# TopHillRobotics/quadruped-robot

Hardware: AMD Instinct MI355X
Metric: MPC+WBC control ticks/s (batched robots) (higher is better)
Workload: dtype f32 assembly / f64 QP+WBC

## Files before the change

quadruped-robot_amd/csrc/qrgpu_api.hip:

```cpp
#include <hip/hip_runtime.h>
#include <hip/hip_ext.h>
#include <cmath>
#include <cstdio>
#include <cstdlib>
#include <cstring>
#include <mutex>
#include <string>

#include "qrgpu_ctx.h"
#include "qr_wbc_model.h"

hipError_t create_side_stream(hipStream_t *s)
{
    int least = 0, greatest = 0;
    if (hipDeviceGetStreamPriorityRange(&least, &greatest) == hipSuccess && greatest != least)
        return hipStreamCreateWithPriority(s, hipStreamNonBlocking, greatest);
    return hipStreamCreateWithFlags(s, hipStreamNonBlocking);
}

static void lane_destroy(Lane &L);

int lane_create(qrgpu_ctx *c, Lane &L, bool own_stream, bool masked)
{
    if (L.d_order) return QRGPU_OK;
    L.own_stream = own_stream; L.masked = own_stream && masked;
    const size_t nb = (size_t)c->max_batch;
    auto zalloc = [](auto **p, size_t bytes) { return hipMalloc((void **)p, bytes) == hipSuccess && hipMemset(*p, 0, bytes) == hipSuccess; };
    bool ok = hipMalloc(&L.d_order, sizeof(int) * 2 * nb) == hipSuccess && zalloc(&L.d_rescue, sizeof(int) * (nb + 2)) && zalloc(&L.d_pre, sizeof(int) * (2 * nb + 4)) &&
              zalloc(&L.d_skip, nb) && hipHostMalloc((void **)&L.h_pre_count, 4 * sizeof(int), hipHostMallocMapped) == hipSuccess &&
              hipHostGetDevicePointer((void **)&L.d_pre_hint, L.h_pre_count, 0) == hipSuccess && zalloc(&L.d_started, sizeof(int)) &&
              ((own_stream && !masked) || masked || create_side_stream(&L.side_stream) == hipSuccess) && zalloc(&L.d_done_flag, sizeof(unsigned) * nb) && zalloc(&L.d_qhead, 16 * sizeof(int)) &&
              zalloc(&L.d_planned_done, sizeof(int)) && zalloc(&L.d_go, (1 + QR_ABORT_RING) * sizeof(int)) && zalloc(&L.d_lane_done, sizeof(int)) && zalloc(&L.d_main_done, sizeof(int)) && zalloc(&L.d_rescue_taken, 4 * sizeof(int)) &&
              hipMalloc(&L.d_cmd_tick, sizeof(float) * 12 * nb) == hipSuccess &&
              hipEventCreateWithFlags(&L.ev_fork, hipEventDisableTiming) == hipSuccess && hipEventCreateWithFlags(&L.ev_join, hipEventDisableTiming) == hipSuccess;
    if (ok && own_stream) {
        const uint32_t words = (uint32_t)((c->num_cu + 31) / 32);
        ok = (masked ? (hipExtStreamCreateWithCUMask(&L.stream, words, c->mask16_main) == hipSuccess && hipExtStreamCreateWithCUMask(&L.side_stream, words, c->mask16_side) == hipSuccess)
                     : hipStreamCreateWithFlags(&L.stream, hipStreamNonBlocking) == hipSuccess);
    }
    if (ok && masked) ok = hipMemset(L.d_rescue + 2, 0xff, sizeof(int) * nb) == hipSuccess;
    if (ok) { L.h_pre_count[0] = L.h_pre_count[1] = L.h_pre_count[2] = L.h_pre_count[3] = 0; }
    (void)hipDeviceSynchronize();
    if (!ok) lane_destroy(L);
    return ok ? QRGPU_OK : QRGPU_ERR_ALLOC;
}
static void lane_destroy(Lane &L)
{
    if (L.stream && L.own_stream) { (void)hipStreamSynchronize(L.stream); }
    if (L.side_stream && (!L.own_stream || L.masked)) { (void)hipStreamSynchronize(L.side_stream); hipStreamDestroy(L.side_stream); }
    if (L.stream && L.own_stream) hipStreamDestroy(L.stream);
    (void)hipHostFree(L.h_pre_count);
    for (void *p : {(void *)L.d_order, (void *)L.d_rescue, (void *)L.d_pre, (void *)L.d_skip, (void *)L.d_started, (void *)L.d_done_flag, (void *)L.d_qhead,
                    (void *)L.d_planned_done, (void *)L.d_go, (void *)L.d_lane_done, (void *)L.d_main_done, (void *)L.d_rescue_taken, (void *)L.d_cmd_tick})
        (void)hipFree(p);
    if (L.ev_fork) hipEventDestroy(L.ev_fork);
    if (L.ev_join) hipEventDestroy(L.ev_join);
    L = Lane{};
}

int upload_wbc(qrgpu_ctx *c)
{
    if (!c->wbc_dirty) return QRGPU_OK;
    HIPCHK(c, hipMemcpyAsync(c->d_wbc, c->wbc_host, sizeof(WbcConst) * QRGPU_MAX_TYPES, hipMemcpyHostToDevice, c->stream));
    HIPCHK(c, hipStreamSynchronize(c->stream));
    c->wbc_dirty = false;
    return QRGPU_OK;
}

int launch_wbc(qrgpu_ctx *c, int n, const int *d_type, const float *d_state, const float *d_cmd, float *d_prev, float *d_tau, float *d_qdes, int *d_status,
               const WbcOpts &o)
{
    if (!batch_ok(c, n) || !d_state) return QRGPU_ERR_BAD_ARG;
    if (!o.dbg && (!d_cmd || !d_prev || !d_tau)) return QRGPU_ERR_BAD_ARG;
    if (!(d_type ? ready_mask(c->wbc_ready) != 0 : c->wbc_ready[0])) return QRGPU_ERR_NOT_SETUP;
    HIPCHK(c, hipSetDevice(c->device));
    int rc = upload_wbc(c);
    if (rc) return rc;
    const hipStream_t ws = o.stream ? o.stream : c->stream;
    if (!o.pipe.wbc_done) c->ov_chain = false;
    {
        TimerScope ts(c, 1, ws, !o.pipe.second && o.timed);
        hipLaunchKernelGGL((o.dbg || o.qp || c->d_dbg_cycles_wbc) ? qr_wbc_kernel_dbg : qr_wbc_kernel, dim3(o.grid_wgs > 0 ? o.grid_wgs : 8 * ((n + 7) / 8)), dim3(128), 0, ws, n, c->d_wbc, d_type, d_state,
                           d_cmd ? d_cmd : d_state, d_prev, d_tau, d_qdes, d_status, o.dbg, o.merge, o.status_or, (long long *)c->d_dbg_cycles_wbc, o.fr,
                           ready_mask(c->wbc_ready), o.epilogue, o.qp, o.pipe);
    }
    HIPCHK(c, hipGetLastError());
    return QRGPU_OK;
}

int launch_vmc(qrgpu_ctx *c, int n, const int *d_type_id, const float *d_vmc_in, const float *d_ratio, const float *d_q, float *d_force,
               float *d_tau, int *d_status)
{
    if (!batch_ok(c, n) || !d_vmc_in || !d_force) return QRGPU_ERR_BAD_ARG;
    if (d_tau && !d_q) return QRGPU_ERR_BAD_ARG;
    if (!(d_type_id ? ready_mask(c->vmc_ready) != 0 : c->vmc_ready[0])) return QRGPU_ERR_NOT_SETUP;
    HIPCHK(c, hipSetDevice(c->device));
    VmcLaunch P = c->vmc;
    P.n = n; P.ratio = d_ratio; P.type_ready = ready_mask(c->vmc_ready);
    hipLaunchKernelGGL(qr_vmc_kernel, dim3(8 * ((n + 7) / 8)), dim3(64), 0, c->stream, P, d_type_id, d_vmc_in, d_q, d_force, d_tau, d_status);
    HIPCHK(c, hipGetLastError());
    return QRGPU_OK;
}

extern "C" {

void qrgpu_model_desc_default(qrgpu_model_desc *d)
{
    d->hip_l = 0.08505f; d->upper_l = 0.2f; d->lower_l = 0.2f;
    d->body_size[0] = 0.267f; d->body_size[1] = 0.194f; d->body_size[2] = 0.114f;
    d->kp_body_pos = 100.f; d->kd_body_pos = 10.f; d->kp_body_ori = 100.f; d->kd_body_ori = 10.f;
    d->kp_foot = 500.f; d->kd_foot = 10.f; d->weight_fb = 0.1f; d->weight_fr = 1.f; d->mu = 0.4f;
}

extern char **environ;
static void warn_unknown_env()
{
    static std::once_flag once;
    std::call_once(once, [] {
        static const char *supported[] = {QRGPU_SUPPORTED_ENV};
        static const char *labs[] = {QRGPU_LAB_ENV};
        const bool lab_on = lab_env("QRGPU_LAB") != nullptr;
        for (char **e = environ; e && *e; ++e) {
            if (strncmp(*e, "QRGPU_", 6) != 0 || strncmp(*e, "QRGPU_BENCH_", 12) == 0) continue;
            const char *eq = strchr(*e, '=');
            const std::string name(*e, eq ? (size_t)(eq - *e) : strlen(*e));
            bool ok = false, is_lab = false;
            for (const char *s_ : supported) if (name == s_) ok = true;
            for (const char *s_ : labs) if (name == s_) is_lab = true;
            if (ok || (is_lab && lab_on)) continue;
            if (is_lab) fprintf(stderr, "libqrgpu: %s is a laboratory switch: ignored unless QRGPU_LAB=1 is set (include/qrgpu.h lists the supported ones)\n", name.c_str());
            else fprintf(stderr, "libqrgpu: %s is not an environment switch of this library (include/qrgpu.h lists the supported ones): ignored\n", name.c_str());
        }
    });
}

int qrgpu_create(int device_id, int max_batch, int horizon_max, qrgpu_ctx **out)
{
    if (!out || max_batch <= 0 || horizon_max <= 0 || horizon_max > QRGPU_MAX_HORIZON) return QRGPU_ERR_BAD_ARG;
    warn_unknown_env();
    *out = nullptr;
    int ndev = 0;
    if (hipGetDeviceCount(&ndev) != hipSuccess || device_id < 0 || device_id >= ndev) return QRGPU_ERR_NO_DEVICE;
    if (hipSetDevice(device_id) != hipSuccess) return QRGPU_ERR_NO_DEVICE;
    hipDeviceProp_t prop;
    if (hipGetDeviceProperties(&prop, device_id) != hipSuccess) return QRGPU_ERR_NO_DEVICE;
    if (strncmp(prop.gcnArchName, "gfx950", 6) != 0) return QRGPU_ERR_NO_DEVICE;
    qrgpu_ctx *c = new qrgpu_ctx();
    c->device = device_id; c->max_batch = max_batch; c->horizon_max = horizon_max;
    c->name = prop.name; c->num_cu = prop.multiProcessorCount;
    c->lds_per_cu = (int)prop.maxSharedMemoryPerMultiProcessor;
    if (c->lds_per_cu <= 0) c->lds_per_cu = 160 * 1024;
    const size_t in1 = 28 + 12 * QRGPU_MAX_HORIZON + 4 * QRGPU_MAX_HORIZON + 12 + 37 + 67 + 3;
    static_assert(28 + 12 * QRGPU_MAX_HORIZON + 4 * QRGPU_MAX_HORIZON + 12 + 37 + 67 + 3 <= 512, "staging layout");
    c->zero_copy = !qr_env().single_copies;
    bool stage_ok;
    if (c->zero_copy) {
        void *dp = nullptr;
        stage_ok = hipHostMalloc(&c->h_stage, 640 * sizeof(float), hipHostMallocMapped) == hipSuccess &&
                   hipHostGetDevicePointer(&dp, c->h_stage, 0) == hipSuccess;
        if (stage_ok) {
            memset(c->h_stage, 0, 640 * sizeof(float));
            c->h_in1 = (float *)c->h_stage; c->h_out1 = c->h_in1 + 512; c->h_st1 = (int *)(c->h_in1 + 576);
            c->d_in1 = (float *)dp; c->d_out1 = c->d_in1 + 512; c->d_st1 = (int *)(c->d_in1 + 576);
        }
    } else {
        stage_ok = hipMalloc(&c->d_in1, in1 * sizeof(float)) == hipSuccess && hipMalloc(&c->d_out1, 64 * sizeof(float)) == hipSuccess &&
                   hipMalloc(&c->d_st1, 4 * sizeof(int)) == hipSuccess;
    }
    auto zalloc = [](auto **p, size_t bytes) { return hipMalloc((void **)p, bytes) == hipSuccess && hipMemset(*p, 0, bytes) == hipSuccess; };
    bool ok = stage_ok && hipMalloc(&c->d_wbc, sizeof(WbcConst) * QRGPU_MAX_TYPES) == hipSuccess;
    const size_t nb = (size_t)max_batch;
    ok = ok && zalloc(&c->d_body, sizeof(qrgpu_plant_body_desc) * QRGPU_MAX_TYPES);
    ok = ok && zalloc(&c->d_cost[0], sizeof(int) * nb) && zalloc(&c->d_cost[1], sizeof(int) * nb) && hipMalloc(&c->d_warm, (size_t)QR_WARM_STRIDE * nb) == hipSuccess &&
         hipStreamCreateWithFlags(&c->wbc_stream, hipStreamNonBlocking) == hipSuccess &&
         zalloc(&c->d_main_started, sizeof(int)) && zalloc(&c->d_tick_done, sizeof(int)) && zalloc(&c->d_gate_abort, QR_ABORT_RING * sizeof(int)) &&
         zalloc(&c->d_wbc_finished, sizeof(int)) && zalloc(&c->d_solved, sizeof(unsigned) * nb) && zalloc(&c->d_wbc_done, sizeof(unsigned) * nb) &&
         hipMalloc(&c->d_ftime, sizeof(int) * nb) == hipSuccess;
    ok = ok && lane_create(c, c->lane[0], false) == QRGPU_OK;
    if (!ok) {
        qrgpu_destroy(c);
        return QRGPU_ERR_ALLOC;
    }
    if (hipStreamCreateWithFlags(&c->own_stream, hipStreamNonBlocking) == hipSuccess) c->stream = c->own_stream;
    c->lane[0].stream = c->stream;
    (void)hipDeviceSynchronize();
    memset(&c->mpc, 0, sizeof(c->mpc));
    memset(c->wbc_host, 0, sizeof(c->wbc_host));
    *out = c;
    return QRGPU_OK;
}

void qrgpu_destroy(qrgpu_ctx *c)
{
    if (!c) return;
    hipSetDevice(c->device);
    (void)hipStreamSynchronize(c->stream);
    if (c->wbc_stream) (void)hipStreamSynchronize(c->wbc_stream);
    qrgpu_comm_destroy(c);
    for (int l = 0; l < QR_LANES; ++l) lane_destroy(c->lane[l]);
    for (int k = 0; k < 2; ++k) for (auto &e : c->ev[k]) { hipEventDestroy(e.first); hipEventDestroy(e.second); }
    for (auto &e : c->marks) hipEventDestroy(e);
    if (c->wbc_stream) hipStreamDestroy(c->wbc_stream);
    if (c->wbc_stream_hi) { (void)hipStreamSynchronize(c->wbc_stream_hi); hipStreamDestroy(c->wbc_stream_hi); }
    if (c->own_stream) hipStreamDestroy(c->own_stream);
    for (int k = 0; k < 2; ++k) if (c->ev_call[k]) hipEventDestroy(c->ev_call[k]);
    if (c->h_stage) (void)hipHostFree(c->h_stage);
    else for (void *p : {(void *)c->d_in1, (void *)c->d_out1, (void *)c->d_st1}) (void)hipFree(p);
    for (void *p : {(void *)c->d_wbc, (void *)c->d_body, (void *)c->d_cost[0], (void *)c->d_cost[1], (void *)c->d_warm, (void *)c->d_flops, (void *)c->d_main_started, (void *)c->d_ftime,
                    (void *)c->d_wbc_finished, (void *)c->d_gate_abort, (void *)c->d_solved, (void *)c->d_wbc_done, (void *)c->d_gather_done, (void *)c->d_tick_done,
                    (void *)c->d_timeline, (void *)c->d_tlr, (void *)c->d_sinv_spill, c->d_dbg_cycles, c->d_dbg_cycles_wbc, (void *)c->d_join_dbg})
        (void)hipFree(p);
    delete c;
}

static void forget_history(qrgpu_ctx *c)
{
    for (auto &L : c->lane) { L.lpt_n = 0; L.plan_n = 0; }
    c->cost_n[0] = c->cost_n[1] = 0;
    c->ov_hold = 0;
}
int qrgpu_set_lpt_schedule(qrgpu_ctx *c, int on)
{
    if (!c) return QRGPU_ERR_BAD_ARG;
    c->lpt = on != 0;
    forget_history(c);
    return QRGPU_OK;
}
int qrgpu_set_warm_start(qrgpu_ctx *c, int on)
{
    if (!c) return QRGPU_ERR_BAD_ARG;
    c->warm = on != 0;
    c->warm_n = 0;
    return QRGPU_OK;
}
int qrgpu_mpc_set_hessian_mode(qrgpu_ctx *c, int mode)
{
    if (!c || (mode != QRGPU_HESSIAN_F32 && mode != QRGPU_HESSIAN_BF16X3)) return QRGPU_ERR_BAD_ARG;
    c->mpc.hess_mode = mode;
    return QRGPU_OK;
}
int qrgpu_set_planned_list(qrgpu_ctx *c, int on, int big_nls)
{
    if (!c || big_nls < 0) return QRGPU_ERR_BAD_ARG;
    c->planned = on != 0;
    c->big_nls = big_nls;
    for (auto &L : c->lane) L.plan_n = 0;
    return QRGPU_OK;
}
int qrgpu_set_tick_pipeline(qrgpu_ctx *c, int on)
{
    if (!c) return QRGPU_ERR_BAD_ARG;
    c->pipeline = on != 0;
    return QRGPU_OK;
}
int qrgpu_set_rescue_pass(qrgpu_ctx *c, int on)
{
    if (!c) return QRGPU_ERR_BAD_ARG;
    c->rescue = on != 0;
    for (auto &L : c->lane) L.plan_n = 0;
    return QRGPU_OK;
}
int qrgpu_set_stream(qrgpu_ctx *c, void *s) { if (!c) return QRGPU_ERR_BAD_ARG; c->stream = (hipStream_t)s; c->lane[0].stream = c->stream; c->ov_chain = false; return QRGPU_OK; }
void *qrgpu_get_stream(qrgpu_ctx *c) { return c ? (void *)c->stream : nullptr; }
const char *qrgpu_last_error(const qrgpu_ctx *c) { return c ? c->err.c_str() : "null context"; }
int qrgpu_device_info(const qrgpu_ctx *c, char *name, int len, int *lds)
{
    if (!c) return 0;
    if (name && len > 0) { strncpy(name, c->name.c_str(), len - 1); name[len - 1] = 0; }
    if (lds) *lds = c->lds_per_cu;
    return c->num_cu;
}

int qrgpu_mpc_setup(qrgpu_ctx *c, int type_id, float dt, int horizon, float mu, float fmax, float mass,
                    const float inertia[3], const float weights[12], float alpha)
{
    if (!c || type_id < 0 || type_id >= QRGPU_MAX_TYPES || !inertia || !weights) return QRGPU_ERR_BAD_ARG;
    if (horizon <= 0 || horizon > c->horizon_max) return QRGPU_ERR_BAD_ARG;
    if (c->mpc.horizon != horizon) for (int t = 0; t < QRGPU_MAX_TYPES; ++t) if (t != type_id) c->mpc_ready[t] = false;
    MpcType &T = c->mpc.type[type_id];
    T.dt = dt; T.mu = mu; T.fmax = fmax; T.mass = mass; T.alpha = alpha;
    for (int i = 0; i < 3; ++i) T.inertia[i] = inertia[i];
    for (int i = 0; i < 12; ++i) T.weights[i] = weights[i];
    if (!c->wbc_ready[type_id]) { T.hip_l = 0.08505f; T.upper_l = 0.2f; T.lower_l = 0.2f; }
    c->mpc.horizon = horizon;
    c->mpc_ready[type_id] = true;
    return QRGPU_OK;
}

int qrgpu_wbc_setup(qrgpu_ctx *c, int type_id, const qrgpu_model_desc *desc)
{
    if (!c || type_id < 0 || type_id >= QRGPU_MAX_TYPES || !desc) return QRGPU_ERR_BAD_ARG;
    build_wbc_const(*desc, c->wbc_host[type_id]);
    MpcType &T = c->mpc.type[type_id];
    T.hip_l = desc->hip_l; T.upper_l = desc->upper_l; T.lower_l = desc->lower_l;
    c->wbc_ready[type_id] = true;
    c->wbc_dirty = true;
    return QRGPU_OK;
}

int qrgpu_mpc_solve_batch(qrgpu_ctx *c, int n, const int *d_type_id, const float *d_mpc_state, const float *d_traj,
                          const float *d_gait, const float *d_q, float *d_force, float *d_tau_mpc, int *d_status)
{
// ... 331 lines not shown
```

quadruped-robot_amd/csrc/qrgpu_ctx.h:

```cpp
#pragma once
#include <hip/hip_runtime.h>
#include <cstdlib>
#include <cstring>
#include <string>
#include <utility>
#include <vector>

#include "../../include/qrgpu.h"
#include "qr_device_types.h"
#include "qr_kernels.h"

using namespace qrgpu;

enum MpcVar {
    MPC_MAIN11,
    MPC_LIST11,
    MPC_ONE11,
    MPC_HALF_LIST11,
    MPC_MAIN16,
    MPC_LIST16,
    MPC_TWO16,
    MPC_PERSIST11,
    MPC_PERSIST16,
    MPC_VAR_COUNT,
    MPC_VAR_NONE = -1
};

#define QR_LANES 5
#define QR_ABORT_RING 8
struct Lane {
    hipStream_t stream = nullptr;
    bool own_stream = false;
    hipStream_t side_stream = nullptr;
    hipEvent_t ev_fork = nullptr, ev_join = nullptr;
    int *d_order = nullptr;
    int lpt_n = 0;
    int *d_rescue = nullptr;
    int rescue_parity = 0;
    bool last_rescue_active = false;
    int last_rescue_parity = 0;
    int *d_pre = nullptr;
    unsigned char *d_skip = nullptr;
    int plan_n = 0;
    int *d_pre_hint = nullptr;
    int *h_pre_count = nullptr;
    int plan_sync_left = 0;
    int *d_started = nullptr;
    unsigned started_total = 0;
    int *d_go = nullptr;
    unsigned go_total = 0;
    int plan_epoch = 0;
    int *d_planned_done = nullptr;
    unsigned planned_done_total = 0;
    int *d_qhead = nullptr;
    int qhead_parity = 0;
    int two_hold = 0;
    bool two_probe = false;
    unsigned *d_done_flag = nullptr;
    float *d_cmd_tick = nullptr;
    bool masked = false;
    int *d_lane_done = nullptr;
    int *d_main_done = nullptr; int main_done_total = 0;
    int order_parity = 0;
    const int *order_used = nullptr;
    bool join_recorded = false;
    int last_linger = 0;
    int *d_rescue_taken = nullptr;
    unsigned lane_done_total = 0;
};

struct qrgpu_ctx {
    int device = 0;
    int max_batch = 0;
    int horizon_max = 0;
    hipStream_t stream = nullptr;
    hipStream_t own_stream = nullptr;
    MpcLaunch mpc{};
    bool mpc_ready[QRGPU_MAX_TYPES] = {false, false, false, false};
    bool wbc_ready[QRGPU_MAX_TYPES] = {false, false, false, false};
    VmcLaunch vmc{};
    bool vmc_ready[QRGPU_MAX_TYPES] = {false, false, false, false};
    WbcConst wbc_host[QRGPU_MAX_TYPES];
    WbcConst *d_wbc = nullptr;
    bool wbc_dirty = true;
    qrgpu_plant_body_desc body_host[QRGPU_MAX_TYPES] = {};
    qrgpu_plant_body_desc *d_body = nullptr;
    bool body_ready[QRGPU_MAX_TYPES] = {false, false, false, false};
    bool body_dirty = true;
    qrgpu_stage_reset stage_reset{};
    bool stage_reset_on = false;
    float *d_in1 = nullptr;
    float *d_out1 = nullptr;
    int *d_st1 = nullptr;
    float *h_in1 = nullptr, *h_out1 = nullptr;
    int *h_st1 = nullptr;
    void *h_stage = nullptr;
    bool zero_copy = false;
    int type_stage = 0;
    Lane lane[QR_LANES];
    int *d_cost[2] = {nullptr, nullptr};
    int cost_n[2] = {0, 0};
    double *d_sinv_spill = nullptr;
    bool planned = true;
    int big_nls = 0;
    bool pipeline = true;
    hipStream_t wbc_stream = nullptr;
    int *d_main_started = nullptr;
    unsigned main_started_total = 0;
    unsigned tick_epoch = 0;
    int main_slots[MPC_VAR_COUNT] = {};
    int main_slots_lds[MPC_VAR_COUNT] = {};
    int *d_tick_done = nullptr;
    unsigned tick_done_total = 0;
    bool last_tick_piped = false;
    int *d_gather_done = nullptr;
    unsigned gather_total[2] = {0, 0};
    unsigned gather_joined[2] = {0, 0};
    int *d_gate_abort = nullptr;
    int *d_wbc_finished = nullptr;
    unsigned wbc_finished_total = 0;
    int overlap = 0;
    int ov_next = 0;
    bool ov_chain = false;
    int ov_n = 0;
    unsigned ov_epoch = 0, ov_main_total = 0;
    const void *ov_out[4] = {nullptr, nullptr, nullptr, nullptr};
    const void *ov_prev_ori = nullptr;
    int ov_lane_last = 0;
    int ov_fence_slots = 0;
    int ov_hold = 0;
    bool ov_prev_plan = false;
    hipStream_t wbc_stream_hi = nullptr;
    int ov16_side_cus = 0;
    uint32_t mask16_main[16] = {}, mask16_side[16] = {};
    hipEvent_t ev_call[2] = {nullptr, nullptr};
    int ev_call_last = -1;
    long long *d_join_dbg = nullptr;
    int ov_stats[2] = {0, 0};
    unsigned *d_solved = nullptr;
    unsigned *d_wbc_done = nullptr;
    int *d_tlr = nullptr;
    long long *d_timeline = nullptr;
    int *d_ftime = nullptr;
    bool lpt = true;
    bool rescue = true;
    int epilogue = 0;
    double *d_flops = nullptr;
    bool flops_on = false;
    int flops_n = 0;
    bool warm = true;
    unsigned char *d_warm = nullptr;
    int warm_n = 0;
    bool last_main_persist = false;
    void *d_dbg_cycles_wbc = nullptr;
    void *d_dbg_cycles = nullptr;
    int lds_per_cu = 0, num_cu = 0;
    std::string name;
    std::string err;
    void *comm = nullptr;
    bool comm_owned = false;
    int comm_nranks = 0, comm_rank = 0;
    hipStream_t comm_stream = nullptr;
    hipEvent_t ev_tick = nullptr;
    hipEvent_t ev_gather[2] = {nullptr, nullptr};
    bool ev_gather_pending[2] = {false, false};
    bool timing = false;
    bool timing_paused = false;
    int timing_every = 1;
    unsigned ev_calls[2] = {0, 0};
    std::vector<std::pair<hipEvent_t, hipEvent_t>> ev[2];
    size_t ev_used[2] = {0, 0};
    std::vector<hipEvent_t> marks;
};

inline const char *lab_env(const char *name)
{
    static const bool lab = [] { const char *e = getenv("QRGPU_LAB"); return e && atoi(e) != 0; }();
    return lab ? getenv(name) : nullptr;
}
#define QRGPU_SUPPORTED_ENV "QRGPU_TICK_PIPELINE", "QRGPU_PIPE_GATE_MS", "QRGPU_PLAN_GO_MS", "QRGPU_PIPE_WAIT_US", "QRGPU_OV_WAIT_US", "QRGPU_OV_FAULT", "QRGPU_OV_PLAN_HOLD", "QRGPU_OV16", \
                            "QRGPU_COMM_EVENTS", "QRGPU_SINGLE_COPIES", "QRGPU_PERSIST", "QRGPU_H16_TWO", "QRGPU_H16_TWO_HOLD", "QRGPU_H16_BIG_US", "QRGPU_H16_BIG_STAY_US", \
                            "QRGPU_LIB", "QRGPU_EXTRA_FLAGS", "QRGPU_LAB"
#define QRGPU_LAB_ENV "QRGPU_WBC_CHUNKS", "QRGPU_PLANNED_FORK"

struct QrEnv {
    static int num(const char *e, int dflt) { return e ? atoi(e) : dflt; }
    static long long ms(const char *e) { return 100000LL * (e ? atoll(e) : 50LL); }
    static long long us(const char *e, long long dflt_ticks) { return e ? 100LL * atoll(e) : dflt_ticks; }
    int tick_pipeline = num(getenv("QRGPU_TICK_PIPELINE"), 1);
    long long pipe_gate_ticks = ms(getenv("QRGPU_PIPE_GATE_MS"));
    long long plan_go_ticks = ms(getenv("QRGPU_PLAN_GO_MS"));
    long long pipe_wait_ticks = us(getenv("QRGPU_PIPE_WAIT_US"), 400000LL);
    long long ov_wait_ticks = us(getenv("QRGPU_OV_WAIT_US"), 2000000LL);
    int ov_fault = num(getenv("QRGPU_OV_FAULT"), 0);
    int ov_plan_hold = num(getenv("QRGPU_OV_PLAN_HOLD"), 31);
    bool ov16 = num(getenv("QRGPU_OV16"), 1) != 0;
    int comm_events = num(getenv("QRGPU_COMM_EVENTS"), -1);
    bool single_copies = num(getenv("QRGPU_SINGLE_COPIES"), 0) != 0;
    int persist = num(getenv("QRGPU_PERSIST"), 1);
    int h16_two = num(getenv("QRGPU_H16_TWO"), 1);
    int h16_two_hold = num(getenv("QRGPU_H16_TWO_HOLD"), 31);
    int h16_big_us = num(getenv("QRGPU_H16_BIG_US"), 450);
    int h16_big_stay_us = num(getenv("QRGPU_H16_BIG_STAY_US"), 300);
    int wbc_chunks = num(lab_env("QRGPU_WBC_CHUNKS"), 0);
    int planned_fork = num(lab_env("QRGPU_PLANNED_FORK"), 0);
};
inline const QrEnv &qr_env() { static const QrEnv env{}; return env; }

#define HIPCHK(ctx, call)                                                                    \
    do {                                                                                     \
        hipError_t e_ = (call);                                                              \
        if (e_ != hipSuccess) {                                                              \
            (ctx)->err = std::string(#call) + ": " + hipGetErrorString(e_);                  \
            return QRGPU_ERR_LAUNCH;                                                         \
        }                                                                                    \
    } while (0)


inline int ready_mask(const bool *r) { int m = 0; for (int t = 0; t < QRGPU_MAX_TYPES; ++t) if (r[t]) m |= 1 << t; return m; }

inline bool batch_ok(const qrgpu_ctx *c, int n) { return c && n > 0 && n <= c->max_batch; }

struct DeviceScratch {
    void *p = nullptr;
    DeviceScratch() = default;
    DeviceScratch(const DeviceScratch &) = delete;
    DeviceScratch &operator=(const DeviceScratch &) = delete;
    ~DeviceScratch() { (void)hipFree(p); }
};

struct TimerScope {
    qrgpu_ctx *c; int k; bool on; hipStream_t s;
    TimerScope(qrgpu_ctx *ctx, int kernel, hipStream_t stream = nullptr, bool enabled = true) : c(ctx), k(kernel), on(ctx->timing && enabled), s(stream ? stream : ctx->stream)
    {
        if (on && ctx->timing_every > 1 && (ctx->ev_calls[kernel]++ % (unsigned)ctx->timing_every) != 0) on = false;
        if (!on) return;
        if (c->ev_used[k] == c->ev[k].size()) {
            hipEvent_t a, b;
            if (hipEventCreate(&a) != hipSuccess || hipEventCreate(&b) != hipSuccess) { on = false; return; }
            c->ev[k].push_back({a, b});
        }
        hipEventRecord(c->ev[k][c->ev_used[k]].first, s);
    }
    ~TimerScope()
    {
        if (!on) return;
        hipEventRecord(c->ev[k][c->ev_used[k]].second, s);
        c->ev_used[k]++;
    }
};

struct OvLaunch { unsigned epoch; bool chained; unsigned prev_epoch; bool plan_tick; int *prev_started; unsigned prev_started_total; };

struct MpcOpts {
    int epilogue = 0;
    bool piped = false;
    int lane_id = 0;
    const OvLaunch *ov = nullptr;
};
struct WbcOpts {
    float *dbg = nullptr;
    int merge = 0, status_or = 0;
    const float *fr = nullptr;
    int epilogue = 0;
    float *qp = nullptr;
    hipStream_t stream = nullptr;
    WbcPipe pipe{};
    int grid_wgs = 0;
    bool timed = true;
};
inline MpcIO mpc_io(const int *type_id, const float *state, const float *traj, const float *gait, const float *q, float *force, float *tau, int *status)
{
    MpcIO io{};
    io.type_id = type_id; io.g_state = state; io.g_traj = traj; io.g_gait = gait; io.g_q = q; io.g_force = force; io.g_tau = tau; io.g_status = status;
    return io;
}
int launch_mpc(qrgpu_ctx *c, int n, const MpcIO &arrays, const MpcOpts &opt = MpcOpts{});
int launch_wbc(qrgpu_ctx *c, int n, const int *d_type, const float *d_state, const float *d_cmd, float *d_prev, float *d_tau, float *d_qdes, int *d_status,
               const WbcOpts &opt = WbcOpts{});
int launch_vmc(qrgpu_ctx *c, int n, const int *d_type_id, const float *d_vmc_in, const float *d_ratio, const float *d_q, float *d_force, float *d_tau,
               int *d_status);
int upload_wbc(qrgpu_ctx *c);
hipError_t create_side_stream(hipStream_t *s);
int lane_create(qrgpu_ctx *c, Lane &L, bool own_stream, bool masked = false);

inline bool lane_has_plan(const qrgpu_ctx *c, const Lane &L, int n)
{
    return c->planned && c->rescue && c->lpt && L.plan_n == n && L.h_pre_count[L.rescue_parity] > 0;
}
inline bool list_exceeds_45_percent(const Lane &L, int n)
{
    return L.plan_n == n && 20 * (long long)L.h_pre_count[L.rescue_parity] > 9 * (long long)n;
}
inline bool h16_two_allowed(const qrgpu_ctx *c, int n)
{
    const int two = qr_env().h16_two;
    return two != 0 && n >= (two >= 2 ? 64 : 7 * c->num_cu / 2) && c->rescue && c->planned && c->lpt;
}
```

quadruped-robot_amd/csrc/qrgpu_tick.hip:

```cpp
#include <hip/hip_runtime.h>
#include <hip/hip_ext.h>
#include <cstdio>

#include "qrgpu_ctx.h"

struct TickArgs {
    int n;
    const int *type_id;
    const float *mpc_state, *traj, *gait, *fb_state, *wbc_cmd;
    float *prev_ori, *force, *tau, *qdes;
    int *status;
};

static bool tick_is_piped(qrgpu_ctx *c, int n)
{
    if (!(c->pipeline && qr_env().tick_pipeline != 0 && n >= 64 && !c->d_dbg_cycles && !c->d_dbg_cycles_wbc)) return false;
    hipStreamCaptureStatus cap = hipStreamCaptureStatusNone;
    if (hipStreamIsCapturing(c->stream, &cap) != hipSuccess) { cap = hipStreamCaptureStatusNone; (void)hipGetLastError(); }
    return cap == hipStreamCaptureStatusNone;
}

static bool ov_on_hold(qrgpu_ctx *c, int hold_calls, bool trigger)
{
    if (c->ov_hold > 0) { --c->ov_hold; return true; }
    if (hold_calls > 0 && trigger) { c->ov_hold = hold_calls; return true; }
    return false;
}

static bool tick_overlaps(qrgpu_ctx *c, int n, bool small_h)
{
    if (!c->overlap || c->flops_on) return false;
    if (!(small_h ? (c->lane[1].d_order && c->lane[2].d_order) : (c->lane[3].d_order && c->lane[4].d_order))) return false;
    const Lane &NL = c->lane[(small_h ? 1 : 3) + c->ov_next];
    if (!small_h) return h16_two_allowed(c, n) && !ov_on_hold(c, qr_env().h16_two_hold, list_exceeds_45_percent(NL, n));
    return !ov_on_hold(c, qr_env().ov_plan_hold, lane_has_plan(c, NL, n));
}

static int ov_begin(qrgpu_ctx *c, Lane &LN, const TickArgs &a, bool was_chain, bool small_h, unsigned epoch, unsigned prev_epoch, OvLaunch &ov)
{
    const int n = a.n;
    c->ov_next ^= 1;
    const void *outs[4] = {(const void *)a.force, (const void *)a.tau, (const void *)a.qdes, (const void *)a.status};
    bool distinct = true;
    for (int x = 0; x < 4; ++x) if (outs[x]) for (int y = 0; y < 4; ++y) if (outs[x] == c->ov_out[y]) distinct = false;
    ov.plan_tick = small_h && lane_has_plan(c, LN, n);
    ov.chained = was_chain && c->ov_n == n && c->ov_epoch == prev_epoch && c->ov_prev_ori == (const void *)a.prev_ori && distinct && !ov.plan_tick && !c->ov_prev_plan;
    c->ov_prev_plan = ov.plan_tick;
    const int ev_now = (c->ev_call_last + 1) & 1;
    const int ev_prev = c->ev_call_last;
    HIPCHK(c, hipEventRecord(c->ev_call[ev_now], c->stream));
    if (ov.chained && ev_prev >= 0) {
        HIPCHK(c, hipStreamWaitEvent(LN.stream, c->ev_call[ev_prev], 0));
        Lane &PL = c->lane[c->ov_lane_last];
        hipLaunchKernelGGL(qr_gate2_kernel, dim3(1), dim3(64), 0, LN.stream, c->d_main_started, (int)c->ov_main_total, small_h ? PL.d_started : (int *)nullptr, (int)PL.started_total, (long long)5000000,
                           c->d_timeline ? c->d_timeline + QR_TL_GATES + (epoch & 63u) * 2 : (long long *)nullptr);
        HIPCHK(c, hipGetLastError());
    } else {
        ov.chained = false;
        HIPCHK(c, hipStreamWaitEvent(LN.stream, c->ev_call[ev_now], 0));
    }
    c->ev_call_last = ev_now;
    if (ov.chained) {
        const Lane &PL = c->lane[c->ov_lane_last];
        ov.prev_started = PL.d_started; ov.prev_started_total = PL.started_total - (PL.last_linger < 8 ? PL.last_linger : 8);
    }
    for (int sl = 0; sl < 2; ++sl)
        if (((c->ov_fence_slots >> sl) & 1) && c->ev_gather[sl]) HIPCHK(c, hipStreamWaitEvent(LN.stream, c->ev_gather[sl], 0));
    c->ov_fence_slots = 0;
    for (int x = 0; x < 4; ++x) c->ov_out[x] = outs[x];
    return QRGPU_OK;
}

static WbcOpts tick_wbc_opts(const qrgpu_ctx *c, const TickArgs &a, float *force)
{
    WbcOpts o;
    o.merge = 1; o.status_or = a.status ? 1 : 0; o.fr = force; o.epilogue = c->epilogue;
    return o;
}

static int tick_issue_wbc(qrgpu_ctx *c, Lane &LN, const TickArgs &a, float *force, bool ovl, bool small_h, hipStream_t wbc_stream, unsigned epoch, unsigned wait_epoch,
                          int *gate_abort)
{
    const QrEnv &env = qr_env();
    const int n = a.n;
    const int total_wgs = 8 * ((n + 7) / 8);
    const bool chunked = env.wbc_chunks && !ovl && n >= 4096 && small_h && !c->last_main_persist;
    const int chunk_wgs = chunked ? 1024 : total_wgs;
    const int expect = (int)c->main_started_total;
    const int main_before = (int)(c->main_started_total - (unsigned)total_wgs);
    for (int base = 0; base < total_wgs; base += chunk_wgs) {
        const int wgs = (total_wgs - base < chunk_wgs) ? total_wgs - base : chunk_wgs;
        hipLaunchKernelGGL(qr_gate_kernel, dim3(1), dim3(64), 0, wbc_stream, c->d_main_started, chunked ? main_before + base + wgs : expect, ovl ? 200000000LL : env.pipe_gate_ticks,
                           ovl ? (int *)nullptr : gate_abort, (int)epoch, (int *)nullptr);
        HIPCHK(c, hipGetLastError());
        WbcOpts o = tick_wbc_opts(c, a, force);
        o.stream = wbc_stream; o.grid_wgs = chunked ? wgs : 0; o.timed = base == 0;
        o.pipe.flag = LN.d_done_flag; o.pipe.epoch = epoch;
        o.pipe.gate_abort = ovl ? (int *)nullptr : gate_abort;
        o.pipe.finished = c->d_wbc_finished;
        o.pipe.tlr = c->d_tlr; o.pipe.tl = c->d_timeline;
        o.pipe.order = chunked ? LN.order_used : nullptr;
        o.pipe.wbc_done = ovl ? c->d_wbc_done : nullptr; o.pipe.wait_epoch = wait_epoch; o.pipe.wait_ticks = env.ov_wait_ticks;
        o.pipe.wait_list = ovl ? 1 : 0;
        o.pipe.flag_ticks = env.pipe_wait_ticks;
        o.pipe.slot_base = chunked ? base : 0;
        const int rc = launch_wbc(c, n, a.type_id, a.fb_state, a.wbc_cmd, a.prev_ori, a.tau, a.qdes, a.status, o);
        if (rc) return rc;
    }
    return QRGPU_OK;
}

static int tick_issue_second_pass(qrgpu_ctx *c, Lane &LN, const TickArgs &a, float *force, unsigned epoch, int *gate_abort)
{
    const bool have_list = LN.last_rescue_active;
    WbcOpts o = tick_wbc_opts(c, a, force);
    o.pipe.epoch = epoch;
    o.pipe.list = have_list ? LN.d_rescue + 2 : nullptr; o.pipe.list_count = have_list ? LN.d_rescue + LN.last_rescue_parity : nullptr;
    o.pipe.gate_abort = gate_abort;
// ... 14 lines not shown
    c->gather_joined[0] = c->gather_total[0]; c->gather_joined[1] = c->gather_total[1];
    ++c->tick_done_total; c->last_tick_piped = true;
    return QRGPU_OK;
}

extern "C" {

int qrgpu_tick_batch(qrgpu_ctx *c, int n, const int *d_type_id, const float *d_mpc_state, const float *d_traj,
                     const float *d_gait, const float *d_fb_state, const float *d_wbc_cmd, float *d_prev_ori,
                     float *d_force, float *d_tau, float *d_qdes, int *d_status)
{
    if (!c || !d_fb_state || !d_wbc_cmd || !d_tau || !d_prev_ori) return QRGPU_ERR_BAD_ARG;
    if (n <= 0 || n > c->max_batch) return QRGPU_ERR_BAD_ARG;
    HIPCHK(c, hipSetDevice(c->device));
    c->last_tick_piped = false;
    const bool piped = tick_is_piped(c, n);
    const bool was_chain = c->ov_chain;
    const bool small_h = 4 * c->mpc.horizon <= 44;
    const bool ovl = piped && tick_overlaps(c, n, small_h);
    const int lane_id = ovl ? (small_h ? 1 : 3) + c->ov_next : 0;
    Lane &LN = c->lane[lane_id];
    float *const force = d_force ? d_force : LN.d_cmd_tick;
    const TickArgs a{n, d_type_id, d_mpc_state, d_traj, d_gait, d_fb_state, d_wbc_cmd, d_prev_ori, d_force, d_tau, d_qdes, d_status};
    const MpcIO mpc_arrays = mpc_io(d_type_id, d_mpc_state, d_traj, d_gait, d_fb_state + (size_t)13 * n, force, d_tau, d_status);
    if (!piped) {
        int rc = launch_mpc(c, n, mpc_arrays);
        if (rc) return rc;
        return launch_wbc(c, n, d_type_id, d_fb_state, d_wbc_cmd, d_prev_ori, d_tau, d_qdes, d_status, tick_wbc_opts(c, a, force));
    }
    const unsigned prev_epoch = c->tick_epoch;
    if (++c->tick_epoch >= 0x3fffffffu) c->tick_epoch = 1;
    const unsigned epoch = c->tick_epoch;
    int *const gate_abort = c->d_gate_abort + (epoch & (QR_ABORT_RING - 1));
    const unsigned waited_epoch = (prev_epoch + (qr_env().ov_fault == 1 ? 0x10000000u : 0u)) & 0x3fffffffu;
    OvLaunch ov{epoch, false, waited_epoch, false, nullptr, 0u};
    if (ovl) { const int rc = ov_begin(c, LN, a, was_chain, small_h, epoch, prev_epoch, ov); if (rc) return rc; }
    MpcOpts mo;
    mo.piped = true; mo.lane_id = lane_id; mo.ov = ovl ? &ov : nullptr;
    int rc = launch_mpc(c, n, mpc_arrays, mo);
    if (rc) return rc;
    const hipStream_t wbc_stream = ovl ? c->wbc_stream_hi : c->wbc_stream;
    if (ovl && !ov.chained) HIPCHK(c, hipStreamWaitEvent(wbc_stream, c->ev_call[c->ev_call_last], 0));
    rc = tick_issue_wbc(c, LN, a, force, ovl, small_h, wbc_stream, epoch, (ovl && ov.chained) ? waited_epoch : 0u, gate_abort);
    if (!rc && !ovl) rc = tick_issue_second_pass(c, LN, a, force, epoch, gate_abort);
    if (!rc) rc = tick_issue_join(c, n);
    if (rc) return rc;
    if (ovl) {
        ++c->ov_stats[ov.chained ? 0 : 1];
        c->ov_chain = true; c->ov_n = n; c->ov_epoch = epoch; c->ov_main_total = c->main_started_total; c->ov_prev_ori = (const void *)d_prev_ori; c->ov_lane_last = lane_id;
    }
    return QRGPU_OK;
}

int qrgpu_tick_cadence_batch(qrgpu_ctx *c, int n, const int *d_type_id, const int *d_mpc_updated, const float *d_mpc_state, const float *d_traj,
                             const float *d_gait, const float *d_fb_state, const float *d_wbc_cmd, float *d_prev_ori, float *d_force, float *d_hold,
                             float *d_tau, float *d_qdes, int *d_status)
{
    if (!c || !d_mpc_updated || !d_force || !d_hold) return QRGPU_ERR_BAD_ARG;
    if (!d_mpc_state || !d_traj || !d_gait || !d_fb_state || !d_wbc_cmd || !d_tau || !d_prev_ori) return QRGPU_ERR_BAD_ARG;
    if (n <= 0 || n > c->max_batch) return QRGPU_ERR_BAD_ARG;
    if (!(d_type_id ? (ready_mask(c->mpc_ready) != 0 && ready_mask(c->wbc_ready) != 0) : (c->mpc_ready[0] && c->wbc_ready[0]))) return QRGPU_ERR_NOT_SETUP;
    HIPCHK(c, hipSetDevice(c->device));
    c->last_tick_piped = false;
    const TickArgs a{n, d_type_id, d_mpc_state, d_traj, d_gait, d_fb_state, d_wbc_cmd, d_prev_ori, d_force, d_tau, d_qdes, d_status};
    MpcIO io = mpc_io(d_type_id, d_mpc_state, d_traj, d_gait, d_fb_state + (size_t)13 * n, d_force, d_tau, d_status);
    io.due = d_mpc_updated;
    MpcOpts mo;
    mo.epilogue = c->epilogue;
    int rc = launch_mpc(c, n, io, mo);
    if (rc) return rc;
    CadenceLegs L{};
    for (int t = 0; t < QRGPU_MAX_TYPES; ++t) { L.hip_l[t] = c->mpc.type[t].hip_l; L.upper_l[t] = c->mpc.type[t].upper_l; L.lower_l[t] = c->mpc.type[t].lower_l; }
    L.type_ready = ready_mask(c->mpc_ready);
    hipLaunchKernelGGL(qr_cadence_kernel, dim3((n + 63) / 64), dim3(64), 0, c->stream, n, L, d_type_id, d_mpc_updated, d_mpc_state, d_fb_state, (const float *)d_force, d_hold,
                       d_tau, d_status);
    HIPCHK(c, hipGetLastError());
    WbcOpts o = tick_wbc_opts(c, a, d_force);
    o.pipe.skip = d_mpc_updated;
    return launch_wbc(c, n, d_type_id, d_fb_state, d_wbc_cmd, d_prev_ori, d_tau, d_qdes, d_status, o);
}

}

static int probe_streams(qrgpu_ctx *c, hipStream_t *st, int nst, int npair)
{
    DeviceScratch scratch;
    HIPCHK(c, hipMalloc(&scratch.p, 16 * sizeof(int)));
    int *const d_probe = (int *)scratch.p;
    HIPCHK(c, hipMemset(d_probe, 0, 16 * sizeof(int)));
    HIPCHK(c, hipDeviceSynchronize());
    int k = 0, token = 0;
    for (int a = 0; a < nst; ++a)
        for (int b = 0; b < nst; ++b) {
            if (a == b || (a >= npair && b >= npair)) continue;
            int res = 0;
            for (int attempt = 0; attempt < 2 && res != 1; ++attempt) {
                ++token;
                hipLaunchKernelGGL(qr_probe_wait_kernel, dim3(1), dim3(64), 0, st[a], d_probe + k, d_probe + 8, (long long)2000000, token);
                hipLaunchKernelGGL(qr_probe_set_kernel, dim3(1), dim3(64), 0, st[b], d_probe + k, token);
                HIPCHK(c, hipStreamSynchronize(st[a]));
                HIPCHK(c, hipStreamSynchronize(st[b]));
                HIPCHK(c, hipMemcpy(&res, d_probe + 8, sizeof(int), hipMemcpyDeviceToHost));
                k = (k + 1) & 7;
            }
            if (res != 1) {
                static char msg[320];
                snprintf(msg, sizeof(msg), "qrgpu_set_tick_overlap: two of the context's streams share a hardware queue in this process (set GPU_MAX_HW_QUEUES=8 before the first HIP call); "
                         "overlapped ticks stay off [a launch on stream %d of the set waited for one queued behind it on stream %d]", a, b);
                c->err = msg;
                c->overlap = 0;
                return QRGPU_ERR_NOT_SETUP;
            }
        }
    return QRGPU_OK;
}

extern "C" {

int qrgpu_set_tick_overlap(qrgpu_ctx *c, int on)
{
    if (!c) return QRGPU_ERR_BAD_ARG;
    c->ov_chain = false;
    if (!on) { c->overlap = 0; return QRGPU_OK; }
    HIPCHK(c, hipSetDevice(c->device));
    if (!c->ev_call[0]) for (int k = 0; k < 2; ++k) HIPCHK(c, hipEventCreateWithFlags(&c->ev_call[k], hipEventDisableTiming));
    if (!c->wbc_stream_hi) HIPCHK(c, create_side_stream(&c->wbc_stream_hi));
    const bool want16 = 4 * c->mpc.horizon > 44;
    hipStream_t st[6]; int nst = 0, npair = 0;
    if (!want16) {
        for (int l = 1; l <= 2; ++l) {
            if (lane_create(c, c->lane[l], true) != QRGPU_OK) { c->err = "qrgpu_set_tick_overlap: allocation of a lane failed"; return QRGPU_ERR_ALLOC; }
            c->lane[l].side_stream = c->lane[0].side_stream;
        }
        st[0] = c->lane[1].stream; st[1] = c->lane[2].stream; st[2] = c->wbc_stream_hi; st[3] = c->stream; nst = 4; npair = 2;
    } else if (qr_env().ov16) {
        if (!c->ov16_side_cus) {
            int k = (64 * c->num_cu / 256) & ~31;
            if (k < 32) k = 32;
            if (k > c->num_cu / 2) k = (c->num_cu / 2) & ~31;
            c->ov16_side_cus = k;
            for (int b = 0; b < c->num_cu && b < 512; ++b) { if (b < c->num_cu - k) c->mask16_main[b >> 5] |= 1u << (b & 31); else c->mask16_side[b >> 5] |= 1u << (b & 31); }
        }
        for (int l = 3; l <= 4; ++l)
            if (lane_create(c, c->lane[l], true, true) != QRGPU_OK) { c->err = "qrgpu_set_tick_overlap: allocation of a CU-masked lane failed"; return QRGPU_ERR_ALLOC; }
        st[0] = c->lane[3].stream; st[1] = c->lane[4].stream; st[2] = c->lane[3].side_stream; st[3] = c->lane[4].side_stream; st[4] = c->wbc_stream_hi; st[5] = c->stream; nst = 6; npair = 4;
    } else { c->overlap = 1; return QRGPU_OK; }
    const int rc = probe_streams(c, st, nst, npair);
    if (rc) return rc;
    c->overlap = 1;
    return QRGPU_OK;
}
int qrgpu_tick_fence(qrgpu_ctx *c) { if (!c) return QRGPU_ERR_BAD_ARG; c->ov_chain = false; return QRGPU_OK; }
int qrgpu_tick_overlap_stats(const qrgpu_ctx *c, int *chained, int *unchained)
{
    if (!c) return QRGPU_ERR_BAD_ARG;
    if (chained) *chained = c->ov_stats[0];
    if (unchained) *unchained = c->ov_stats[1];
    return QRGPU_OK;
}

}
```

Measured before the change: 4.588 million.

## Rework overlap lanes: borrow WBC stream, retry stream probing, adaptive plan hold

```diff
diff --git a/quadruped-robot_amd/csrc/qrgpu_api.hip b/quadruped-robot_amd/csrc/qrgpu_api.hip
--- a/quadruped-robot_amd/csrc/qrgpu_api.hip
+++ b/quadruped-robot_amd/csrc/qrgpu_api.hip
@@ -20,36 +20,45 @@
 
 static void lane_destroy(Lane &L);
 
-int lane_create(qrgpu_ctx *c, Lane &L, bool own_stream, bool masked)
-{
-    if (L.d_order) return QRGPU_OK;
-    L.own_stream = own_stream; L.masked = own_stream && masked;
+int lane_create(qrgpu_ctx *c, Lane &L, LaneKind kind, hipStream_t given)
+{
+    if (L.complete) return QRGPU_OK;
+    if ((kind == LANE_BORROW || kind == LANE_CTX) && !given) return QRGPU_ERR_BAD_ARG;
+    lane_destroy(L);
+    if (kind == LANE_CTX) { L.side_stream = given; L.own_side = true; }
+    const bool masked = kind == LANE_MASKED;
     const size_t nb = (size_t)c->max_batch;
-    auto zalloc = [](auto **p, size_t bytes) { return hipMalloc((void **)p, bytes) == hipSuccess && hipMemset(*p, 0, bytes) == hipSuccess; };
+    const hipStream_t fs = c->stream;
+    auto zalloc = [fs](auto **p, size_t bytes) { return hipMalloc((void **)p, bytes) == hipSuccess && hipMemsetAsync(*p, 0, bytes, fs) == hipSuccess; };
     bool ok = hipMalloc(&L.d_order, sizeof(int) * 2 * nb) == hipSuccess && zalloc(&L.d_rescue, sizeof(int) * (nb + 2)) && zalloc(&L.d_pre, sizeof(int) * (2 * nb + 4)) &&
               zalloc(&L.d_skip, nb) && hipHostMalloc((void **)&L.h_pre_count, 4 * sizeof(int), hipHostMallocMapped) == hipSuccess &&
               hipHostGetDevicePointer((void **)&L.d_pre_hint, L.h_pre_count, 0) == hipSuccess && zalloc(&L.d_started, sizeof(int)) &&
-              ((own_stream && !masked) || masked || create_side_stream(&L.side_stream) == hipSuccess) && zalloc(&L.d_done_flag, sizeof(unsigned) * nb) && zalloc(&L.d_qhead, 16 * sizeof(int)) &&
+              zalloc(&L.d_done_flag, sizeof(unsigned) * nb) && zalloc(&L.d_qhead, 16 * sizeof(int)) &&
               zalloc(&L.d_planned_done, sizeof(int)) && zalloc(&L.d_go, (1 + QR_ABORT_RING) * sizeof(int)) && zalloc(&L.d_lane_done, sizeof(int)) && zalloc(&L.d_main_done, sizeof(int)) && zalloc(&L.d_rescue_taken, 4 * sizeof(int)) &&
               hipMalloc(&L.d_cmd_tick, sizeof(float) * 12 * nb) == hipSuccess &&
               hipEventCreateWithFlags(&L.ev_fork, hipEventDisableTiming) == hipSuccess && hipEventCreateWithFlags(&L.ev_join, hipEventDisableTiming) == hipSuccess;
-    if (ok && own_stream) {
+    if (ok && kind == LANE_BORROW) L.stream = given;
+    if (ok && kind == LANE_OWN) { ok = hipStreamCreateWithFlags(&L.stream, hipStreamNonBlocking) == hipSuccess; L.own_stream = ok; }
+    if (ok && masked) {
         const uint32_t words = (uint32_t)((c->num_cu + 31) / 32);
-        ok = (masked ? (hipExtStreamCreateWithCUMask(&L.stream, words, c->mask16_main) == hipSuccess && hipExtStreamCreateWithCUMask(&L.side_stream, words, c->mask16_side) == hipSuccess)
-                     : hipStreamCreateWithFlags(&L.stream, hipStreamNonBlocking) == hipSuccess);
-    }
-    if (ok && masked) ok = hipMemset(L.d_rescue + 2, 0xff, sizeof(int) * nb) == hipSuccess;
+        ok = hipExtStreamCreateWithCUMask(&L.stream, words, c->mask16_main) == hipSuccess; L.own_stream = ok;
+        if (ok) { ok = hipExtStreamCreateWithCUMask(&L.side_stream, words, c->mask16_side) == hipSuccess; L.own_side = ok; }
+    }
+    if (ok && (kind == LANE_BORROW || kind == LANE_OWN)) L.side_stream = c->lane[0].side_stream;
+    L.masked = masked;
+    if (ok && masked) ok = hipMemsetAsync(L.d_rescue + 2, 0xff, sizeof(int) * nb, fs) == hipSuccess;
     if (ok) { L.h_pre_count[0] = L.h_pre_count[1] = L.h_pre_count[2] = L.h_pre_count[3] = 0; }
-    (void)hipDeviceSynchronize();
-    if (!ok) lane_destroy(L);
-    return ok ? QRGPU_OK : QRGPU_ERR_ALLOC;
+    if (hipStreamSynchronize(fs) != hipSuccess) ok = false;
+    if (!ok) { lane_destroy(L); return QRGPU_ERR_ALLOC; }
+    L.complete = true;
+    return QRGPU_OK;
 }
 static void lane_destroy(Lane &L)
 {
-    if (L.stream && L.own_stream) { (void)hipStreamSynchronize(L.stream); }
-    if (L.side_stream && (!L.own_stream || L.masked)) { (void)hipStreamSynchronize(L.side_stream); hipStreamDestroy(L.side_stream); }
+    if (L.stream && L.own_stream) (void)hipStreamSynchronize(L.stream);
+    if (L.side_stream && L.own_side) { (void)hipStreamSynchronize(L.side_stream); hipStreamDestroy(L.side_stream); }
     if (L.stream && L.own_stream) hipStreamDestroy(L.stream);
-    (void)hipHostFree(L.h_pre_count);
+    if (L.h_pre_count) (void)hipHostFree(L.h_pre_count);
     for (void *p : {(void *)L.d_order, (void *)L.d_rescue, (void *)L.d_pre, (void *)L.d_skip, (void *)L.d_started, (void *)L.d_done_flag, (void *)L.d_qhead,
                     (void *)L.d_planned_done, (void *)L.d_go, (void *)L.d_lane_done, (void *)L.d_main_done, (void *)L.d_rescue_taken, (void *)L.d_cmd_tick})
         (void)hipFree(p);
@@ -167,8 +176,12 @@
         stage_ok = hipMalloc(&c->d_in1, in1 * sizeof(float)) == hipSuccess && hipMalloc(&c->d_out1, 64 * sizeof(float)) == hipSuccess &&
                    hipMalloc(&c->d_st1, 4 * sizeof(int)) == hipSuccess;
     }
-    auto zalloc = [](auto **p, size_t bytes) { return hipMalloc((void **)p, bytes) == hipSuccess && hipMemset(*p, 0, bytes) == hipSuccess; };
-    bool ok = stage_ok && hipMalloc(&c->d_wbc, sizeof(WbcConst) * QRGPU_MAX_TYPES) == hipSuccess;
+    hipStream_t side = nullptr;
+    const bool side_ok = create_side_stream(&side) == hipSuccess;
+    if (hipStreamCreateWithFlags(&c->own_stream, hipStreamNonBlocking) == hipSuccess) c->stream = c->own_stream;
+    const hipStream_t fs = c->stream;
+    auto zalloc = [fs](auto **p, size_t bytes) { return hipMalloc((void **)p, bytes) == hipSuccess && hipMemsetAsync(*p, 0, bytes, fs) == hipSuccess; };
+    bool ok = stage_ok && side_ok && hipMalloc(&c->d_wbc, sizeof(WbcConst) * QRGPU_MAX_TYPES) == hipSuccess;
     const size_t nb = (size_t)max_batch;
     ok = ok && zalloc(&c->d_body, sizeof(qrgpu_plant_body_desc) * QRGPU_MAX_TYPES);
     ok = ok && zalloc(&c->d_cost[0], sizeof(int) * nb) && zalloc(&c->d_cost[1], sizeof(int) * nb) && hipMalloc(&c->d_warm, (size_t)QR_WARM_STRIDE * nb) == hipSuccess &&
@@ -176,14 +189,14 @@
          zalloc(&c->d_main_started, sizeof(int)) && zalloc(&c->d_tick_done, sizeof(int)) && zalloc(&c->d_gate_abort, QR_ABORT_RING * sizeof(int)) &&
          zalloc(&c->d_wbc_finished, sizeof(int)) && zalloc(&c->d_solved, sizeof(unsigned) * nb) && zalloc(&c->d_wbc_done, sizeof(unsigned) * nb) &&
          hipMalloc(&c->d_ftime, sizeof(int) * nb) == hipSuccess;
-    ok = ok && lane_create(c, c->lane[0], false) == QRGPU_OK;
+    if (ok) ok = lane_create(c, c->lane[0], LANE_CTX, side) == QRGPU_OK;
+    else if (side) hipStreamDestroy(side);
+    ok = ok && hipStreamSynchronize(fs) == hipSuccess;
     if (!ok) {
         qrgpu_destroy(c);
         return QRGPU_ERR_ALLOC;
     }
-    if (hipStreamCreateWithFlags(&c->own_stream, hipStreamNonBlocking) == hipSuccess) c->stream = c->own_stream;
     c->lane[0].stream = c->stream;
-    (void)hipDeviceSynchronize();
     memset(&c->mpc, 0, sizeof(c->mpc));
     memset(c->wbc_host, 0, sizeof(c->wbc_host));
     *out = c;
@@ -217,7 +230,7 @@
 {
     for (auto &L : c->lane) { L.lpt_n = 0; L.plan_n = 0; }
     c->cost_n[0] = c->cost_n[1] = 0;
-    c->ov_hold = 0;
+    c->ov_hold = OvHold{}; c->ov16_hold = 0;
 }
 int qrgpu_set_lpt_schedule(qrgpu_ctx *c, int on)
 {
diff --git a/quadruped-robot_amd/csrc/qrgpu_ctx.h b/quadruped-robot_amd/csrc/qrgpu_ctx.h
--- a/quadruped-robot_amd/csrc/qrgpu_ctx.h
+++ b/quadruped-robot_amd/csrc/qrgpu_ctx.h
@@ -1,4 +1,35 @@
 #pragma once
+
+struct OvHold {
+    bool on = false;
+    int held = 0;
+    int clear = 0;
+    int blind = 0;
+};
+inline bool ov_hold_step(OvHold &H, int min_hold, int clear_need, bool trigger, int lane0_count, bool *armed = nullptr, bool *resumed = nullptr)
+{
+    if (armed) *armed = false;
+    if (resumed) *resumed = false;
+    if (min_hold <= 0) { H = OvHold{}; return false; }
+    if (!H.on) {
+        if (H.blind > 0) { --H.blind; return false; }
+        if (!trigger) return false;
+        H.on = true; H.held = 1; H.clear = 0;
+        if (armed) *armed = true;
+        return true;
+    }
+    H.clear = lane0_count == 0 ? H.clear + 1 : 0;
+    if (H.held >= min_hold && H.clear >= (clear_need > 0 ? clear_need : 1)) {
+        H = OvHold{};
+        H.blind = 1;
+        if (resumed) *resumed = true;
+        return false;
+    }
+    ++H.held;
+    return true;
+}
+
+#ifndef QRGPU_CTX_HOLD_ONLY
 #include <hip/hip_runtime.h>
 #include <cstdlib>
 #include <cstring>
@@ -32,6 +63,8 @@
     hipStream_t stream = nullptr;
     bool own_stream = false;
     hipStream_t side_stream = nullptr;
+    bool own_side = false;
+    bool complete = false;
     hipEvent_t ev_fork = nullptr, ev_join = nullptr;
     int *d_order = nullptr;
     int lpt_n = 0;
@@ -128,7 +161,8 @@
     const void *ov_prev_ori = nullptr;
     int ov_lane_last = 0;
     int ov_fence_slots = 0;
-    int ov_hold = 0;
+    OvHold ov_hold;
+    int ov16_hold = 0;
     bool ov_prev_plan = false;
     hipStream_t wbc_stream_hi = nullptr;
     int ov16_side_cus = 0;
@@ -178,7 +212,7 @@
     static const bool lab = [] { const char *e = getenv("QRGPU_LAB"); return e && atoi(e) != 0; }();
     return lab ? getenv(name) : nullptr;
 }
-#define QRGPU_SUPPORTED_ENV "QRGPU_TICK_PIPELINE", "QRGPU_PIPE_GATE_MS", "QRGPU_PLAN_GO_MS", "QRGPU_PIPE_WAIT_US", "QRGPU_OV_WAIT_US", "QRGPU_OV_FAULT", "QRGPU_OV_PLAN_HOLD", "QRGPU_OV16", \
+#define QRGPU_SUPPORTED_ENV "QRGPU_TICK_PIPELINE", "QRGPU_PIPE_GATE_MS", "QRGPU_PLAN_GO_MS", "QRGPU_PIPE_WAIT_US", "QRGPU_OV_WAIT_US", "QRGPU_OV_FAULT", "QRGPU_OV_PLAN_HOLD", "QRGPU_OV_PLAN_CLEAR", "QRGPU_OV16", \
                             "QRGPU_COMM_EVENTS", "QRGPU_SINGLE_COPIES", "QRGPU_PERSIST", "QRGPU_H16_TWO", "QRGPU_H16_TWO_HOLD", "QRGPU_H16_BIG_US", "QRGPU_H16_BIG_STAY_US", \
                             "QRGPU_LIB", "QRGPU_EXTRA_FLAGS", "QRGPU_LAB"
 #define QRGPU_LAB_ENV "QRGPU_WBC_CHUNKS", "QRGPU_PLANNED_FORK"
@@ -194,6 +228,7 @@
     long long ov_wait_ticks = us(getenv("QRGPU_OV_WAIT_US"), 2000000LL);
     int ov_fault = num(getenv("QRGPU_OV_FAULT"), 0);
     int ov_plan_hold = num(getenv("QRGPU_OV_PLAN_HOLD"), 31);
+    int ov_plan_clear = num(getenv("QRGPU_OV_PLAN_CLEAR"), 24);
     bool ov16 = num(getenv("QRGPU_OV16"), 1) != 0;
     int comm_events = num(getenv("QRGPU_COMM_EVENTS"), -1);
     bool single_copies = num(getenv("QRGPU_SINGLE_COPIES"), 0) != 0;
@@ -282,7 +317,8 @@
                int *d_status);
 int upload_wbc(qrgpu_ctx *c);
 hipError_t create_side_stream(hipStream_t *s);
-int lane_create(qrgpu_ctx *c, Lane &L, bool own_stream, bool masked = false);
+enum LaneKind { LANE_CTX, LANE_BORROW, LANE_OWN, LANE_MASKED };
+int lane_create(qrgpu_ctx *c, Lane &L, LaneKind kind, hipStream_t given = nullptr);
 
 inline bool lane_has_plan(const qrgpu_ctx *c, const Lane &L, int n)
 {
@@ -297,3 +333,4 @@
     const int two = qr_env().h16_two;
     return two != 0 && n >= (two >= 2 ? 64 : 7 * c->num_cu / 2) && c->rescue && c->planned && c->lpt;
 }
+#endif
diff --git a/quadruped-robot_amd/csrc/qrgpu_tick.hip b/quadruped-robot_amd/csrc/qrgpu_tick.hip
--- a/quadruped-robot_amd/csrc/qrgpu_tick.hip
+++ b/quadruped-robot_amd/csrc/qrgpu_tick.hip
@@ -20,10 +20,25 @@
     return cap == hipStreamCaptureStatusNone;
 }
 
-static bool ov_on_hold(qrgpu_ctx *c, int hold_calls, bool trigger)
-{
-    if (c->ov_hold > 0) { --c->ov_hold; return true; }
-    if (hold_calls > 0 && trigger) { c->ov_hold = hold_calls; return true; }
+static bool ov_on_hold(qrgpu_ctx *c, const Lane &NL, int n)
+{
+    Lane &L0 = c->lane[0];
+    const int lane0_count = (c->ov_hold.on && L0.plan_n == n) ? L0.h_pre_count[L0.rescue_parity] : -1;
+    bool armed = false, resumed = false;
+    const bool held = ov_hold_step(c->ov_hold, qr_env().ov_plan_hold, qr_env().ov_plan_clear, lane_has_plan(c, NL, n), lane0_count, &armed, &resumed);
+    if (armed) {
+        L0.h_pre_count[0] = L0.h_pre_count[1] = -1;
+    }
+    if (resumed) {
+        for (int l = 1; l <= 2; ++l) { Lane &L = c->lane[l]; L.plan_n = 0; L.h_pre_count[0] = L.h_pre_count[1] = 0; L.plan_sync_left = 2; }
+    }
+    return held;
+}
+
+static bool ov16_on_hold(qrgpu_ctx *c, int hold_calls, bool trigger)
+{
+    if (c->ov16_hold > 0) { --c->ov16_hold; return true; }
+    if (hold_calls > 0 && trigger) { c->ov16_hold = hold_calls; return true; }
     return false;
 }
 
@@ -32,8 +47,8 @@
     if (!c->overlap || c->flops_on) return false;
     if (!(small_h ? (c->lane[1].d_order && c->lane[2].d_order) : (c->lane[3].d_order && c->lane[4].d_order))) return false;
     const Lane &NL = c->lane[(small_h ? 1 : 3) + c->ov_next];
-    if (!small_h) return h16_two_allowed(c, n) && !ov_on_hold(c, qr_env().h16_two_hold, list_exceeds_45_percent(NL, n));
-    return !ov_on_hold(c, qr_env().ov_plan_hold, lane_has_plan(c, NL, n));
+    if (!small_h) return h16_two_allowed(c, n) && !ov16_on_hold(c, qr_env().h16_two_hold, list_exceeds_45_percent(NL, n));
+    return !ov_on_hold(c, NL, n);
 }
 
 static int ov_begin(qrgpu_ctx *c, Lane &LN, const TickArgs &a, bool was_chain, bool small_h, unsigned epoch, unsigned prev_epoch, OvLaunch &ov)
@@ -214,13 +229,13 @@
 
 }
 
-static int probe_streams(qrgpu_ctx *c, hipStream_t *st, int nst, int npair)
+static int probe_streams(qrgpu_ctx *c, hipStream_t *st, int nst, int npair, int *bad)
 {
     DeviceScratch scratch;
     HIPCHK(c, hipMalloc(&scratch.p, 16 * sizeof(int)));
     int *const d_probe = (int *)scratch.p;
-    HIPCHK(c, hipMemset(d_probe, 0, 16 * sizeof(int)));
-    HIPCHK(c, hipDeviceSynchronize());
+    HIPCHK(c, hipMemsetAsync(d_probe, 0, 16 * sizeof(int), c->stream));
+    HIPCHK(c, hipStreamSynchronize(c->stream));
     int k = 0, token = 0;
     for (int a = 0; a < nst; ++a)
         for (int b = 0; b < nst; ++b) {
@@ -232,7 +247,8 @@
                 hipLaunchKernelGGL(qr_probe_set_kernel, dim3(1), dim3(64), 0, st[b], d_probe + k, token);
                 HIPCHK(c, hipStreamSynchronize(st[a]));
                 HIPCHK(c, hipStreamSynchronize(st[b]));
-                HIPCHK(c, hipMemcpy(&res, d_probe + 8, sizeof(int), hipMemcpyDeviceToHost));
+                HIPCHK(c, hipMemcpyAsync(&res, d_probe + 8, sizeof(int), hipMemcpyDeviceToHost, c->stream));
+                HIPCHK(c, hipStreamSynchronize(c->stream));
                 k = (k + 1) & 7;
             }
             if (res != 1) {
@@ -241,6 +257,7 @@
                          "overlapped ticks stay off [a launch on stream %d of the set waited for one queued behind it on stream %d]", a, b);
                 c->err = msg;
                 c->overlap = 0;
+                bad[0] = a; bad[1] = b;
                 return QRGPU_ERR_NOT_SETUP;
             }
         }
@@ -260,9 +277,8 @@
     const bool want16 = 4 * c->mpc.horizon > 44;
     hipStream_t st[6]; int nst = 0, npair = 0;
     if (!want16) {
-        for (int l = 1; l <= 2; ++l) {
-            if (lane_create(c, c->lane[l], true) != QRGPU_OK) { c->err = "qrgpu_set_tick_overlap: allocation of a lane failed"; return QRGPU_ERR_ALLOC; }
-            c->lane[l].side_stream = c->lane[0].side_stream;
+        if (lane_create(c, c->lane[1], LANE_BORROW, c->wbc_stream) != QRGPU_OK || lane_create(c, c->lane[2], LANE_OWN) != QRGPU_OK) {
+            c->err = "qrgpu_set_tick_overlap: allocation of a lane failed"; return QRGPU_ERR_ALLOC;
         }
         st[0] = c->lane[1].stream; st[1] = c->lane[2].stream; st[2] = c->wbc_stream_hi; st[3] = c->stream; nst = 4; npair = 2;
     } else if (qr_env().ov16) {
@@ -274,10 +290,24 @@
             for (int b = 0; b < c->num_cu && b < 512; ++b) { if (b < c->num_cu - k) c->mask16_main[b >> 5] |= 1u << (b & 31); else c->mask16_side[b >> 5] |= 1u << (b & 31); }
         }
         for (int l = 3; l <= 4; ++l)
-            if (lane_create(c, c->lane[l], true, true) != QRGPU_OK) { c->err = "qrgpu_set_tick_overlap: allocation of a CU-masked lane failed"; return QRGPU_ERR_ALLOC; }
+            if (lane_create(c, c->lane[l], LANE_MASKED) != QRGPU_OK) { c->err = "qrgpu_set_tick_overlap: allocation of a CU-masked lane failed"; return QRGPU_ERR_ALLOC; }
         st[0] = c->lane[3].stream; st[1] = c->lane[4].stream; st[2] = c->lane[3].side_stream; st[3] = c->lane[4].side_stream; st[4] = c->wbc_stream_hi; st[5] = c->stream; nst = 6; npair = 4;
     } else { c->overlap = 1; return QRGPU_OK; }
-    const int rc = probe_streams(c, st, nst, npair);
+    int rc = QRGPU_OK, bad[2] = {-1, -1};
+    hipStream_t parked[4]; int nparked = 0;
+    for (int attempt = 0;; ++attempt) {
+        rc = probe_streams(c, st, nst, npair, bad);
+        if (rc != QRGPU_ERR_NOT_SETUP || want16 || attempt == 4) break;
+        const int l = (bad[0] == 1 || bad[1] == 1) ? 2 : ((bad[0] == 0 || bad[1] == 0) ? 1 : 0);
+        if (!l) break;
+        Lane &L = c->lane[l];
+        hipStream_t fresh = nullptr;
+        if (hipStreamSynchronize(L.stream) != hipSuccess || hipStreamCreateWithFlags(&fresh, hipStreamNonBlocking) != hipSuccess) break;
+        if (L.own_stream) parked[nparked++] = L.stream;
+        L.stream = fresh; L.own_stream = true;
+        st[l - 1] = fresh;
+    }
+    for (int k = 0; k < nparked; ++k) hipStreamDestroy(parked[k]);
     if (rc) return rc;
     c->overlap = 1;
     return QRGPU_OK;
```

Result: slower. 4.528 million (-1.3%).
